# Polochon-street/bliss

Hardware: AMD Instinct MI355X
Metric: songs/sec bl_analyze (3-min 44.1kHz s16) + 10k x 10k distance-matrix sec (higher is better)
Workload: dtype f64; 1 GPU; configs[2] shard: 8192 synthetic 180-s 44.1 kHz s16 stereo songs/GPU resident (260.1 GB), 8192 total; step = analyze + all-gather + row-block distance; songs_per_gpu=8192, parallelism=shard1, fir_mode=2

## Files before the change

### bliss_amd/csrc/bl_env_kernels.hip

```cpp
#include <hip/hip_runtime.h>
#include <atomic>
#include <algorithm>
#include <stdlib.h>

#include "bl_launch.h"
#include "bl_fft_tan.h"
#include "bl_metric.h"
#include "bl_fir.h"
#include "bl_tail.h"

#define EV_CWAVES 7
#define EV_TILE (4 * EV_CWAVES)
#define EV_TROW 258

template <int CTRL> __device__ __forceinline__ double bl_dpp_f64(double v) {
  const unsigned long long b = __double_as_longlong(v);
  const int lo = __builtin_amdgcn_update_dpp(0, (int)(unsigned)(b & 0xFFFFFFFFull), CTRL, 0xF, 0xF, true);
  const int hi = __builtin_amdgcn_update_dpp(0, (int)(unsigned)(b >> 32), CTRL, 0xF, 0xF, true);
  return __longlong_as_double(((unsigned long long)(unsigned)hi << 32) | (unsigned)lo);
}

template <int CTRL> __device__ __forceinline__ double bl_dpp_f64_old(double old, double v) {
  const unsigned long long b = __double_as_longlong(v), o = __double_as_longlong(old);
  const int lo = __builtin_amdgcn_update_dpp((int)(unsigned)(o & 0xFFFFFFFFull), (int)(unsigned)(b & 0xFFFFFFFFull),
// ... 131 lines not shown
        if (ln == 0) flags[8] = st;
        psum = sum;
        if (live && !own) {
          energies[sg.env_off + w] = sum;
          lc[sg.env_off + w] = bl_tail_compress((double)sum, tb.log101);
        }
        stamp(st - 1, 2);
      }
    }
    return;
  }

  auto phase = [&](int k) {
    const int pr = (PRIO >> (4 * k)) & 3;
    if (pr == 0) __builtin_amdgcn_s_setprio(0);
    else if (pr == 1) __builtin_amdgcn_s_setprio(1);
    else if (pr == 2) __builtin_amdgcn_s_setprio(2);
    else __builtin_amdgcn_s_setprio(3);
  };
  double *buf = reinterpret_cast<double *>(smem) + wave * EV3_SLOTS;
  const int mean = st.mean;
  const double rcp = st.rcp, rcp_lo = st.rcp_lo;
  const double kappa = st.kappa;
  auto nrm = [&](int k) -> double { return FIR_MODE == 2 ? (double)k : bl_norm(k, rcp, rcp_lo); };
  const int r0 = run_begin(u0 + wave), r1 = run_begin(u0 + wave + 1);
  constexpr bool EV3_TAN = FIR_MODE != 0;
  double t1[16];
  bl_fft16_fold<double> fold;
  c2d w1r[16];
  if (EV3_TAN) {
    const bl_fft_tan_lane<double> *tl = reinterpret_cast<const bl_fft_tan_lane<double> *>(tb.tan_lane) + l;
    t1[0] = 0.0;
#pragma unroll
    for (int k1 = 1; k1 < 16; ++k1) {
      t1[k1] = tl->t1[k1];
      asm volatile("" : "+v"(t1[k1]));
    }
    fold = tl->fold;
#define EV3_PIN(A, N) _Pragma("unroll") for (int i = 0; i < N; ++i) asm volatile("" : "+v"(A[i]));
    EV3_PIN(fold.rb, 4) EV3_PIN(fold.rc, 4) EV3_PIN(fold.rd, 4) EV3_PIN(fold.fb, 4) EV3_PIN(fold.fc, 2) EV3_PIN(fold.g, 3)
#undef EV3_PIN
  } else {
#pragma unroll
    for (int k1 = 1; k1 < 16; ++k1) {
      w1r[k1] = tw256[k1 * 16 + l];
      asm volatile("" : "+v"(w1r[k1].re), "+v"(w1r[k1].im));
    }
  }
  typedef int ev_v4i __attribute__((ext_vector_type(4)));
  unsigned cp[4][2];
  ev_v4i ini0, ini2, ini4;
  if (FIR_MODE == 2) {
    bl_firi_tap_planes(l, g, cp);
#pragma unroll
    for (int j = 0; j < 4; ++j) asm volatile("" : "+v"(cp[j][0]), "+v"(cp[j][1]));
    int k0, k2, k4;
    bl_firi_const(mean, &k0, &k2, &k4);
    ini0 = ev_v4i{k0, k0, k0, k0};
    ini2 = ev_v4i{k2, k2, k2, k2};
    ini4 = ev_v4i{k4, k4, k4, k4};
  }
  int base5 = (4 * r0) % 5;

  if (r0 < r1) {
    const int s0 = 1024 * r0 + 4 * ln;
    double r[20];
#pragma unroll
    for (int u = 0; u < 5; ++u) {
      const int i0 = s0 - 16 + 4 * u;
      const bool ok = i0 >= 0 && i0 + 4 <= n_used;
      const uint2 v = *reinterpret_cast<const uint2 *>(p + (ok ? i0 : 0));
      const unsigned w[2] = {ok ? v.x : 0u, ok ? v.y : 0u};
#pragma unroll
      for (int k = 0; k < 2; ++k) {
        const int lo = (int)(short)(w[k] & 0xFFFFu), hi = (int)(short)(w[k] >> 16);
        r[4 * u + 2 * k] = ok ? nrm(lo - mean) : 0.0;
        r[4 * u + 2 * k + 1] = ok ? nrm(hi - mean) : 0.0;
      }
    }
    double *dst = buf + base5 * EV3_BLK + EV3_ROW(ln >> 2) + EV3_UNIT(2 * (ln & 3));
#pragma unroll
    for (int i = 0; i < 4; ++i) {
#define XW(m) r[i + 16 - (m)]
      dst[EV3_UNIT(i >> 1) + (i & 1)] = BL_FIR_SEL(FIR_MODE, XW);
#undef XW
    }
  }

  uint4 pre[4];
  short preh;
#if defined(__HIP_DEVICE_COMPILE__) && !defined(__gfx950__)
#error "k_env_windows3: the raw-buffer descriptor and its range check are written for gfx950"
#endif
  const __amdgpu_buffer_rsrc_t prs =
      __builtin_amdgcn_make_buffer_rsrc(const_cast<int16_t *>(p), 0, (int)(2u * (unsigned)n_used), 0x00020000);
  unsigned voff = 2u * (unsigned)(1024 * r0 + 240 + (FIR_MODE == 2 ? 16 * l + 8 * g : 16 * ln));
  unsigned voffh = 2u * (unsigned)(1024 * r0 + 256 * g + l);
  typedef unsigned ev_v4u __attribute__((__vector_size__(16)));
  auto fetch = [&]() {
#pragma unroll
    for (int u = 0; u < 4; ++u) {
      const ev_v4u v = __builtin_amdgcn_raw_buffer_load_b128(prs, (int)(voff + (FIR_MODE == 2 ? 512u : 16u) * u), 0, 0);
      pre[u] = make_uint4(v[0], v[1], v[2], v[3]);
    }
    preh = (short)__builtin_amdgcn_raw_buffer_load_b16(prs, (int)voffh, 0, 0);
    voff += 2048u;
    voffh += 2048u;
  };
  fetch();
  double held[8];
#pragma unroll
  for (int k0 = 0; k0 < 8; ++k0) held[k0] = 0.0;
  auto publish_held_only = [&]() {
    while (__builtin_amdgcn_readfirstlane(flags[8]) < seq - 1) __builtin_amdgcn_s_sleep(1);
    ev_lds_acquire();
    double *tg = terms + (4 * wave + g) * EV_TROW;
#pragma unroll
    for (int k0 = 0; k0 < 8; ++k0)
      if (k0 < 7 || l != 15) tg[256 - l - 16 * k0] = held[k0];
    ev_wave_sync();
  };
  for (int s = 0; s < steps; ++s) {
    ++seq;
    const int rho = r0 + s;
    if (rho >= r1) {
      publish_held_only();
      if (ln == 0) flags[wave] = seq;
      continue;
    }
    stamp(s, 0);
    phase(0);
    double yv[16], yh;
    const int kh = (int)preh - mean;
    if (FIR_MODE == 2) {
      ev_v4i acc[4][5];
#pragma unroll
      for (int t = 0; t < 4; ++t) {
        const unsigned w[4] = {pre[t].x, pre[t].y, pre[t].z, pre[t].w};
        unsigned lp[2], hp[2];
        bl_firi_sample_planes(w, lp, hp);
        const ev_v4i smp = {(int)lp[0], (int)lp[1], (int)hp[0], (int)hp[1]};
        const ev_v4i zero = {0, 0, 0, 0};
#define EV3_W64(A, B) (long)(((unsigned long long)(B) << 32) | (unsigned long long)(A))
#define EV3_TAP2(J) ev_v4i{(int)cp[(J) + 1][0], (int)cp[(J) + 1][1], (int)cp[J][0], (int)cp[J][1]}
        acc[t][0] = __builtin_amdgcn_mfma_i32_16x16x32_i8(EV3_W64(cp[0][0], cp[0][1]), EV3_W64(lp[0], lp[1]), ini0, 0, 0, 0);
        acc[t][1] = __builtin_amdgcn_mfma_i32_16x16x64_i8(EV3_TAP2(0), smp, zero, 0, 0, 0);
        acc[t][2] = __builtin_amdgcn_mfma_i32_16x16x64_i8(EV3_TAP2(1), smp, ini2, 0, 0, 0);
        acc[t][3] = __builtin_amdgcn_mfma_i32_16x16x64_i8(EV3_TAP2(2), smp, zero, 0, 0, 0);
        acc[t][4] = __builtin_amdgcn_mfma_i32_16x16x32_i8(EV3_W64(cp[3][0], cp[3][1]), EV3_W64(hp[0], hp[1]), ini4, 0, 0, 0);
#undef EV3_W64
#undef EV3_TAP2
      }
      fetch();
#pragma unroll
      for (int t = 0; t < 4; ++t)
#pragma unroll
        for (int r = 0; r < 4; ++r)
          yv[4 * t + r] = bl_firi_combine(acc[t][0][r], acc[t][1][r], acc[t][2][r], acc[t][3][r], acc[t][4][r]);
#define KH(m) __builtin_amdgcn_update_dpp(0, kh, 0x110 + (m), 0xF, 0xF, true)
      const double hp_[9] = {(double)kh ,
                             (double)(KH(1) + KH(15)), (double)(KH(2) + KH(14)), (double)(KH(3) + KH(13)),
                             (double)(KH(4) + KH(12)), (double)(KH(5) + KH(11)), (double)(KH(6) + KH(10)),
                             (double)(KH(7) + KH(9)), (double)KH(8)};
#undef KH
#define XP(m) hp_[m]
      yh = BL_FIR_INT_P(XP);
#undef XP
    } else {
      double r[32];
#pragma unroll
      for (int u = 0; u < 4; ++u) {
        const unsigned w[4] = {pre[u].x, pre[u].y, pre[u].z, pre[u].w};
#pragma unroll
        for (int k = 0; k < 4; ++k) {
          const int lo = (int)(short)(w[k] & 0xFFFFu), hi = (int)(short)(w[k] >> 16);
          r[8 * u + 2 * k] = nrm(lo - mean);
          r[8 * u + 2 * k + 1] = nrm(hi - mean);
        }
      }
      const double xh = nrm(kh);
      fetch();
#pragma unroll
      for (int i = 0; i < 16; ++i) {
#define XR(m) r[i + 16 - (m)]
        yv[i] = BL_FIR_SEL(FIR_MODE, XR);
#undef XR
      }
      double hx[17];
      hx[0] = xh;
      hx[1] = bl_dpp_f64<0x111>(xh);  hx[2] = bl_dpp_f64<0x112>(xh);  hx[3] = bl_dpp_f64<0x113>(xh);
      hx[4] = bl_dpp_f64<0x114>(xh);  hx[5] = bl_dpp_f64<0x115>(xh);  hx[6] = bl_dpp_f64<0x116>(xh);
      hx[7] = bl_dpp_f64<0x117>(xh);  hx[8] = bl_dpp_f64<0x118>(xh);  hx[9] = bl_dpp_f64<0x119>(xh);
      hx[10] = bl_dpp_f64<0x11A>(xh); hx[11] = bl_dpp_f64<0x11B>(xh); hx[12] = bl_dpp_f64<0x11C>(xh);
      hx[13] = bl_dpp_f64<0x11D>(xh); hx[14] = bl_dpp_f64<0x11E>(xh); hx[15] = bl_dpp_f64<0x11F>(xh);
      hx[16] = 0.0;
#define XH(m) hx[m]
      yh = BL_FIR_SEL(FIR_MODE, XH);
#undef XH
    }
    const int xa = base5 + g, xb = xa + 1;
    const int pa = xa >= 5 ? xa - 5 : xa, pb = xb >= 5 ? xb - 5 : xb;
    double *blk_a = buf + pa * EV3_BLK, *blk_b = buf + pb * EV3_BLK;
    stamp(s, 1);
    phase(1);
    ev_wave_sync();
    if (FIR_MODE == 2) {
#pragma unroll
      for (int t = 0; t < 4; ++t) {
        const int xt = base5 + t + 1, pt = xt >= 5 ? xt - 5 : xt;
        double *d = buf + pt * EV3_BLK + EV3_ROW(l) + EV3_UNIT(2 * g);
#pragma unroll
        for (int r = 0; r < 4; ++r) d[EV3_UNIT(r >> 1) + (r & 1)] = yv[4 * t + r];
      }
    } else {
#pragma unroll
      for (int i = 0; i < 16; ++i) blk_b[EV3_ROW(l) + EV3_UNIT(i >> 1) + (i & 1)] = yv[i];
    }
    buf[EV3_HEADS + ln] = yh;
    ev_wave_sync();
    double re[16], im[16];
    {
      const int off = EV3_ROW(l >> 3) + EV3_UNIT(l & 7);
      const double *ia = blk_a + off, *ib = blk_b + off;
      const double *i0 = l < 8 ? buf + EV3_HEADS + 16 * g + 2 * l : ia;
      re[0] = i0[0];
      im[0] = i0[1];
#pragma unroll
      for (int m1 = 1; m1 < 8; ++m1) { re[m1] = ia[EV3_ROW(2 * m1)]; im[m1] = ia[EV3_ROW(2 * m1) + 1]; }
#pragma unroll
      for (int m1 = 8; m1 < 16; ++m1) { re[m1] = ib[EV3_ROW(2 * (m1 - 8))]; im[m1] = ib[EV3_ROW(2 * (m1 - 8)) + 1]; }
    }
    ev_wave_sync();
    stamp(s, 2);
    phase(2);
    if (EV3_TAN) {
      bl_fft512_pass1_tan(re, im, t1);
    } else {
      bl_fft16(re, im);
#pragma unroll
      for (int k1 = 1; k1 < 16; ++k1) bl_cmul(re[bl_pos16(k1)], im[bl_pos16(k1)], w1r[k1].re, w1r[k1].im);
    }
    stamp(s, 3);
    phase(3);
    double *xg = blk_a;
    const double2 *xrow = reinterpret_cast<const double2 *>(xg + l * 18);
#pragma unroll
    for (int k1 = 0; k1 < 16; ++k1) xg[k1 * 18 + l] = re[bl_pos16(k1)];
    ev_wave_sync();
#pragma unroll
    for (int q = 0; q < 8; ++q) { const double2 v = xrow[q]; re[2 * q] = v.x; re[2 * q + 1] = v.y; }
    ev_wave_sync();
#pragma unroll
    for (int k1 = 0; k1 < 16; ++k1) xg[k1 * 18 + l] = im[bl_pos16(k1)];
    ev_wave_sync();
#pragma unroll
    for (int q = 0; q < 8; ++q) { const double2 v = xrow[q]; im[2 * q] = v.x; im[2 * q + 1] = v.y; }
    ev_wave_sync();
    stamp(s, 4);
    phase(4);
    double *tg = terms + (4 * wave + g) * EV_TROW;
    stamp(s, 5);
    phase(5);
    while (__builtin_amdgcn_readfirstlane(flags[8]) < seq - 1) {}
    ev_lds_acquire();
    stamp(s, 6);
#pragma unroll
    for (int k0 = 0; k0 < 8; ++k0)
      if (k0 < 7 || l != 15) tg[256 - l - 16 * k0] = held[k0];
    if (EV3_TAN) bl_fft16_folded(re, im, fold);
    else bl_fft16(re, im);
    double mir7 = 0.0;
#pragma unroll
    for (int k0 = 0; k0 < 8; ++k0) {
      const double sr = re[bl_pos16(15 - k0)], si = im[bl_pos16(15 - k0)];
      const double zr = k0 ? re[bl_pos16(16 - k0)] : re[bl_pos16(0)];
      const double zi = k0 ? im[bl_pos16(16 - k0)] : im[bl_pos16(0)];
      const double pr = bl_dpp_f64_old<0x111>(zr, bl_dpp_f64<0x140>(sr));
      const double pi = bl_dpp_f64_old<0x111>(zi, bl_dpp_f64<0x140>(si));
      double own;
      if (FIR_MODE == 2)
        bl_fft512_power1_sq<double>(re[bl_pos16(k0)], im[bl_pos16(k0)], pr, pi, tw512[l + 16 * k0], kappa, own, held[k0]);
      else if (EV3_TAN)
        bl_fft512_power1_tan<double, false>(re[bl_pos16(k0)], im[bl_pos16(k0)], pr, pi, tw512[l + 16 * k0], own, held[k0]);
      else
        bl_fft512_power1<double, false>(re[bl_pos16(k0)], im[bl_pos16(k0)], pr, pi, tw512[l + 16 * k0], own, held[k0]);
      tg[l + 16 * k0] = own;
      if (k0 == 7) mir7 = held[7];
    }
    const double mr = re[bl_pos16(8)], mi = im[bl_pos16(8)];
    const double mid = (FIR_MODE == 2 ? 2.0 * kappa : 4.0) * __builtin_fma(mr, mr, mi * mi);
    if (l == 0) tg[128] = mid;
    if (l == 15) tg[129] = mir7;
    ev_wave_sync();
    if (ln == 0) flags[wave] = seq;
    stamp(s, 7);
    base5 = base5 == 0 ? 4 : base5 - 1;
  }
  ++seq;
  publish_held_only();
  if (ln == 0) flags[wave] = seq;
}

#define BL_TAIL_OMAX 48

__global__ __launch_bounds__(192) void k_env_tail(const bl_dsong *__restrict__ songs,
                                                  const double *__restrict__ lc, int n_songs,
                                                  bl_amd_song_result *res, int what) {
  __shared__ double yblk[2][38 * 64];
  __shared__ double oblk[2][BL_TAIL_OMAX * 64];
  __shared__ int ocnt[2][64];
  __shared__ double rings_ab[29 * 64];
  __shared__ double rings_c[19 * 64];
  __shared__ int flag_mem[4];
  typedef __attribute__((address_space(3))) volatile int lds_vint;
  lds_vint *flags = (lds_vint *)flag_mem;
  __builtin_amdgcn_s_setprio(3);
  const int wave = __builtin_amdgcn_readfirstlane(threadIdx.x >> 6), lane = threadIdx.x & 63;
  const int song = blockIdx.x * 64 + lane;
  const bool valid = song < n_songs;
  bl_dsong sg;
  if (valid) sg = songs[song];
  else { sg.nb_frames = 0; sg.n_windows = 0; sg.env_off = 0; sg.n = 1; sg.duration = 1; }
  const int N = 2 * sg.nb_frames;
  int maxN = N;
#pragma unroll
  for (int off = 32; off > 0; off >>= 1) maxN = max(maxN, __shfl_xor(maxN, off));
  if (threadIdx.x < 4) flags[threadIdx.x] = 0;
  __syncthreads();
  const int n_blocks = (maxN + 37) / 38;

  if (wave == 0) {
    bl_tail_iir a;
    a.init();
    const double *mylc = lc + sg.env_off;
    const int nw = sg.n_windows;
    auto fetch = [&](int kb_, double (&dst)[19]) {
#pragma unroll
      for (int q = 0; q < 19; ++q) dst[q] = mylc[max(min(19 * kb_ + q, nw - 1), 0)];
    };
    auto block = [&](int kb, double (&cur)[19], double (&fut)[19]) {
      if (kb >= n_blocks) return;
      fetch(kb + 2, fut);
      double *yo = yblk[kb & 1] + lane;
      double ye[38];
#pragma unroll
      for (int q = 0; q < 19; ++q) a.pair(19 * kb + q < nw ? cur[q] : 0.0, ye[2 * q], ye[2 * q + 1]);
      while (__builtin_amdgcn_readfirstlane(flags[1]) < kb - 1) __builtin_amdgcn_s_sleep(1);
      ev_lds_acquire();
#pragma unroll
      for (int q = 0; q < 38; ++q) yo[q * 64] = ye[q];
      ev_lds_release();
      bl_wave_sync();
      if (lane == 0) flags[0] = kb + 1;
    };
    double pa[19], pb[19], pc[19];
    fetch(0, pa);
    fetch(1, pb);
    for (int kb = 0; kb < n_blocks; kb += 3) {
      block(kb, pa, pc);
      block(kb + 1, pb, pa);
      block(kb + 2, pc, pb);
    }
    return;
  }

  if (wave == 1) {
    bl_tail_ab t;
    t.init(sg.nb_frames, rings_ab + lane, 64);
    for (int kb = 0; kb < n_blocks; ++kb) {
      while (__builtin_amdgcn_readfirstlane(flags[0]) < kb + 1) __builtin_amdgcn_s_sleep(1);
      while (__builtin_amdgcn_readfirstlane(flags[3]) < kb - 1) __builtin_amdgcn_s_sleep(1);
      ev_lds_acquire();
      const double *yin = yblk[kb & 1] + lane;
      const int j = 38 * kb;
      bl_tail_fifo f;
      f.base = oblk[kb & 1] + lane;
      f.stride = 64;
      f.count = 0;
      if (bl_tail_ab::chunk_ok(j, N)) {
        t.fast_chunk38(yin, 64, f.base, 64);
        f.count = 38;
      } else if (j < N) {
        for (int q = 0; q < 38; ++q) {
          const int jj = j + q;
          if (jj < N) {
            t.step(jj, yin[q * 64], f);
            if (jj == N - 1) t.finish(f);
          }
        }
      }
      ocnt[kb & 1][lane] = f.count;
      ev_lds_release();
      bl_wave_sync();
      if (lane == 0) { flags[1] = kb + 1; flags[2] = kb + 1; }
    }
    if (valid) {
      bl_amd_song_result *r = res + sg.out_idx;
      r->atk_sum = t.atk;
      r->v.attack = bl_tail_attack(t.atk, sg.n);
    }
    return;
  }

  bl_tail_c c;
  c.init(sg.nb_frames, rings_c + lane, 64);
  for (int kb = 0; kb < n_blocks; ++kb) {
    while (__builtin_amdgcn_readfirstlane(flags[2]) < kb + 1) __builtin_amdgcn_s_sleep(1);
    ev_lds_acquire();
    const double *oin = oblk[kb & 1] + lane;
    const int cnt = ocnt[kb & 1][lane];
    if (cnt == 38 && c.chunk_ok()) {
      c.fast_chunk38(oin, 64);
    } else {
      for (int q = 0; q < BL_TAIL_OMAX; ++q)
        if (q < cnt) c.push(oin[q * 64]);
    }
    if (valid && c.taken == N && cnt > 0) c.finish();
    ev_lds_release();
    bl_wave_sync();
    if (lane == 0) flags[3] = kb + 1;
  }
  if (!valid) return;
  bl_amd_song_result *r = res + sg.out_idx;
  r->beat = c.beat();
  r->v.tempo = bl_tail_tempo(c.beat(), sg.duration);
  (void)what;
}


static long long *g_env_probe = nullptr;
#ifdef BL_AMD_MEASURE

static int g_env_variant = -1;
extern "C" __attribute__((visibility("default"))) int bl_amd_measure_env(int variant, void *d_probe) {
  g_env_variant = variant;
  g_env_probe = static_cast<long long *>(d_probe);
  return BL_OK;
}
#endif

static std::atomic<int> g_fir_mode{-1};
int blk_fir_mode() {
  int m = g_fir_mode.load(std::memory_order_relaxed);
  if (m < 0) {
    const char *e = getenv("BL_AMD_FIR_FUSED");
    m = e && *e ? atoi(e) : BL_FIR_FUSED_DEFAULT;
  }
  return m < 0 || m > 2 ? BL_FIR_FUSED_DEFAULT : m;
}
extern "C" int bl_amd_fir_mode(void) { return blk_fir_mode(); }
extern "C" int bl_amd_set_fir_mode(int mode) {
  if (mode < -1 || mode > 2) return BL_UNEXPECTED;
  g_fir_mode.store(mode, std::memory_order_relaxed);
  return BL_OK;
}

#define EV_X_BOTH(T) EV_X(2, T, false) EV_X(2, T, true)
#ifdef BL_AMD_MEASURE
#define EV_INSTANCES EV_X(0, BL_ENV_PRIO, false) EV_X(1, BL_ENV_PRIO, false) EV_X_BOTH(BL_ENV_PRIO) EV_PRIO_TABS(EV_X_BOTH)
#else
#define EV_INSTANCES EV_X(0, BL_ENV_PRIO, false) EV_X(1, BL_ENV_PRIO, false) EV_X(2, BL_ENV_PRIO, false)
#endif

int blk_env_configure_device(void) {
#define EV_X(M, T, P)                                                                                    \
  BL_HIP_CHECK(hipFuncSetAttribute(reinterpret_cast<const void *>(k_env_windows3<M, T, P>),              \
                                   hipFuncAttributeMaxDynamicSharedMemorySize, EV3_LDS_BYTES));
  EV_INSTANCES
#undef EV_X
  return BL_OK;
}

int blk_env_windows(const blk_analyze_args &a, int fir_mode, int first, int count, int maxn) {
  Mark m(a.mark, a.mark_user, PK_ENV, a.stream);
  const int gx2 = grid_x_for(std::max(1, (2 * (maxn / 512)) / (4 * 4 * EV_CWAVES)), count, 2, a.n_cu);
  const dim3 grid(gx2, count), block(64 * (EV_CWAVES + 1));
  int prio = BL_ENV_PRIO;
  bool probe = false;
#ifdef BL_AMD_MEASURE
  if (fir_mode == 2 && g_env_variant >= 0) {
    prio = g_env_variant & 0xFFFFFF;
    probe = (g_env_variant >> 24) != 0;
  }
#endif
#define EV_X(M, T, P)                                                                                    \
  if (fir_mode == (M) && prio == (T) && probe == (P)) {                                                  \
    hipLaunchKernelGGL((k_env_windows3<M, T, P>), grid, block, EV3_LDS_BYTES, a.stream, a.pcm,           \
                       a.songs + first, a.stats + first, a.tb, a.energies, a.lc, g_env_probe);           \
    return BL_OK;                                                                                        \
  }
  EV_INSTANCES
#undef EV_X
  return BL_UNEXPECTED;
}

void blk_env_tail(const blk_analyze_args &a, hipStream_t s, int first, int count) {
  Mark m(a.mark, a.mark_user, PK_TAIL, s);
  hipLaunchKernelGGL(k_env_tail, dim3((count + 63) / 64), dim3(192), 0, s, a.songs + first, a.lc, count,
                     a.results, a.what);
}
```

### bliss_amd/csrc/bl_tail.h

```cpp
#ifndef BL_TAIL_H_
#define BL_TAIL_H_

#if defined(__HIPCC__)
#include <hip/hip_runtime.h>
#define BL_THD __host__ __device__ __forceinline__
#else
#include <math.h>
#define BL_THD inline
#endif

#define BL_BOX 19
#define BL_BOX_HALF 10

#define BL_BUT_B0 1.9510e-05
#define BL_BUT_B1 1.1706e-04
#define BL_BUT_B2 2.9266e-04
#define BL_BUT_B3 3.9021e-04
#define BL_BUT_A0 1.00000
#define BL_BUT_A1 (-4.59007)
#define BL_BUT_A2 8.91034
#define BL_BUT_A3 (-9.34191)
#define BL_BUT_A4 5.56998
#define BL_BUT_A5 (-1.78845)
#define BL_BUT_A6 0.24136

BL_THD double bl_div_const(double x, double c, double rc) {
  const double q0 = x * rc;
  const double r0 = __builtin_fma(-q0, c, x);
  return __builtin_fma(r0, rc, q0);
}
#define BL_DIV19(x) bl_div_const((x), 19.0, 1.0 / 19.0)
#define BL_DIV10(x) bl_div_const((x), 10.0, 1.0 / 10.0)

struct bl_peaks {
  double p1, p2;
  int beat, i;
  BL_THD void init() { p1 = 0; p2 = 0; beat = 0; i = 0; }
  BL_THD void push(double v) {
    if (i >= 2) {
      const float epsilon = 0.000001f;
      double dl = p1 - p2, dr = p1 - v;
      if (dl > epsilon && dr > epsilon) beat++;
    }
    p2 = p1;
    p1 = v;
    ++i;
  }
};

template <bool KEEP_OLD> struct bl_box19 {
  double run;
  int N, t, s19, s10;
  BL_THD void init(int n) { run = 0; N = n; t = 0; s19 = 0; s10 = 0; }

  template <typename SINK>
  BL_THD void push(double v, double old, double *ring, double *olds, int stride, SINK &sink) {
    if (t < BL_BOX) {
      run += v;
    } else {
      run -= ring[s19 * stride];
      run += v;
    }
    ring[s19 * stride] = v;
    if (KEEP_OLD) olds[s10 * stride] = old;
    if (t <= 8) {
      sink.push(BL_DIV19(old));
    } else if (t >= BL_BOX - 1 && t <= N - 2) {
      sink.push(BL_DIV19(run));
    }
    ++t;
    s19 = s19 == BL_BOX - 1 ? 0 : s19 + 1;
    s10 = s10 == 9 ? 0 : s10 + 1;
  }

  template <typename SINK>
  BL_THD void finish(const double *ring, const double *olds, int stride, SINK &sink) {
    double acc = KEEP_OLD ? olds[((N - 10) % 10) * stride] : 0.0;
    for (int k = N - BL_BOX; k < N; ++k) acc += ring[(k % BL_BOX) * stride];
    sink.push(BL_DIV19(acc));
    for (int i = N - 9; i < N; ++i) {
      double old = KEEP_OLD ? olds[(i % 10) * stride] : 0.0;
      sink.push(BL_DIV19(old));
    }
  }
};

struct bl_tail_stage2 {
  bl_box19<false> box;
  bl_peaks peaks;
  double *ring;
  int stride;
  BL_THD void push(double v) { box.push(v, 0.0, ring, (double *)0, stride, peaks); }
};

struct bl_tail {
  double x1, x2, x3, x4, x5, x6;
  double y1, y2, y3, y4, y5, y6;
  double atk;
  bl_box19<true> box1;
  bl_tail_stage2 st2;
  double *ring1, *olds1;
  int stride, N;

  BL_THD void init(int nb_frames, double *scratch, int stride_) {
    x1 = x2 = x3 = x4 = x5 = x6 = 0;
    y1 = y2 = y3 = y4 = y5 = y6 = 0;
    atk = 0;
    N = 2 * nb_frames;
    stride = stride_;
    ring1 = scratch;
    olds1 = scratch + 19 * stride_;
    st2.ring = scratch + 29 * stride_;
    st2.stride = stride_;
    box1.init(N);
    st2.box.init(N);
    st2.peaks.init();
  }

  BL_THD void step(int j, double x) {
    double d = 0;
    d += BL_BUT_B0 * x;
    d += BL_BUT_B1 * x1;
    d += BL_BUT_B2 * x2;
    d += BL_BUT_B3 * x3;
    d += BL_BUT_B2 * x4;
    d += BL_BUT_B1 * x5;
    d += BL_BUT_B0 * x6;
    double c = 0;
    c += BL_BUT_A1 * y1;
    c += BL_BUT_A2 * y2;
    c += BL_BUT_A3 * y3;
    c += BL_BUT_A4 * y4;
    c += BL_BUT_A5 * y5;
    c += BL_BUT_A6 * y6;
    const double y = (d - c) / BL_BUT_A0;
    double dj;
    if (j == 0) dj = y;
    else { dj = y - y1; dj = dj > 0 ? dj : 0; }
    const float lambda = 0.8f;
    const double wa = (1 - lambda) * y + BL_DIV10(lambda * 172 * dj);
    x6 = x5; x5 = x4; x4 = x3; x3 = x2; x2 = x1; x1 = x;
    y6 = y5; y5 = y4; y4 = y3; y3 = y2; y2 = y1; y1 = y;
    double ss = 0;
    if (j <= N - 2) { atk += wa; ss = wa; }
    box1.push(ss, wa, ring1, olds1, stride, st2);
  }

  BL_THD void finish() {
    box1.finish(ring1, olds1, stride, st2);
    st2.box.finish(st2.ring, (const double *)0, stride, st2.peaks);
  }

  BL_THD int beat() const { return st2.peaks.beat; }
};

struct bl_tail_iir {
  double x2, x4, x6;
  double y1, y2, y3, y4, y5, y6;
  BL_THD void init() { x2 = x4 = x6 = 0; y1 = y2 = y3 = y4 = y5 = y6 = 0; }
  BL_THD double feedback(double d) {
    double c = 0;
    c += BL_BUT_A1 * y1;
    c += BL_BUT_A2 * y2;
    c += BL_BUT_A3 * y3;
    c += BL_BUT_A4 * y4;
    c += BL_BUT_A5 * y5;
    c += BL_BUT_A6 * y6;
    const double y = (d - c) / BL_BUT_A0;
    y6 = y5; y5 = y4; y4 = y3; y3 = y2; y2 = y1; y1 = y;
    return y;
  }
  BL_THD void pair(double x, double &y_even, double &y_odd) {
    double d = BL_BUT_B0 * x;
    d += BL_BUT_B2 * x2;
    d += BL_BUT_B2 * x4;
    d += BL_BUT_B0 * x6;
    y_even = feedback(d);
    double e = BL_BUT_B1 * x;
    e += BL_BUT_B3 * x2;
    e += BL_BUT_B1 * x4;
    y_odd = feedback(e);
    x6 = x4; x4 = x2; x2 = x;
  }
};

struct bl_tail_fifo {
  double *base;
  int stride, count;
  BL_THD void push(double v) {
    base[count * stride] = v;
    ++count;
  }
};

struct bl_tail_ab {
  double yp;
  double atk;
  bl_box19<true> box1;
  double *ring1, *olds1;
  int stride, N;

  BL_THD void init(int nb_frames, double *scratch, int stride_) {
    yp = 0;
    atk = 0;
    N = 2 * nb_frames;
    stride = stride_;
    ring1 = scratch;
    olds1 = scratch + 19 * stride_;
    box1.init(N);
  }

  BL_THD static bool steady(int j, int n) { return (j & 1) == 0 && j >= 40 && j + 1 <= n - 12; }
  BL_THD static bool chunk_ok(int j, int n) { return steady(j, n) && steady(j + 36, n); }

  BL_THD double weighted(double y, double dj) {
    const float lambda = 0.8f;
    return (1 - lambda) * y + BL_DIV10(lambda * 172 * dj);
  }

  template <typename SINK> BL_THD void step(int j, double y, SINK &sink) {
    double dj;
    if (j == 0) dj = y;
    else { dj = y - yp; dj = dj > 0 ? dj : 0; }
    const double wa = weighted(y, dj);
    yp = y;
    double ss = 0;
    if (j <= N - 2) { atk += wa; ss = wa; }
    box1.push(ss, wa, ring1, olds1, stride, sink);
  }
  template <typename SINK> BL_THD void finish(SINK &sink) { box1.finish(ring1, olds1, stride, sink); }

  template <int P> BL_THD double stage_a(double y) {
    double dj = y - yp;
    dj = dj > 0 ? dj : 0;
    const double wa = weighted(y, dj);
    yp = y;
    atk += wa;
    return wa;
  }
  template <int P> BL_THD double stage_b(double wa, double (&ra)[BL_BOX]) {
    box1.run -= ra[P];
    box1.run += wa;
    ra[P] = wa;
    return BL_DIV19(box1.run);
  }
  template <int T>
  BL_THD void reg_pipe(const double *yin, int ystride, double *o1out, int ostride, double (&ra)[BL_BOX],
                       double (&wa)[2]) {
    if constexpr (T < 2 * BL_BOX + 1) {
      if constexpr (T >= 1) o1out[(T - 1) * ostride] = stage_b<(T - 1) % BL_BOX>(wa[(T - 1) % 2], ra);
      if constexpr (T < 2 * BL_BOX) wa[T % 2] = stage_a<T % BL_BOX>(yin[T * ystride]);
      reg_pipe<T + 1>(yin, ystride, o1out, ostride, ra, wa);
    }
  }

  BL_THD void fast_chunk38(const double *yin, int ystride, double *o1out, int ostride) {
    double ra[BL_BOX];
    {
      int sa = box1.s19;
#pragma unroll
      for (int k = 0; k < BL_BOX; ++k) {
        ra[k] = ring1[sa * stride];
        sa = sa == BL_BOX - 1 ? 0 : sa + 1;
      }
    }
    double wa[2];
    reg_pipe<0>(yin, ystride, o1out, ostride, ra, wa);
    {
      int sa = box1.s19;
#pragma unroll
      for (int k = 0; k < BL_BOX; ++k) {
        ring1[sa * stride] = ra[k];
        sa = sa == BL_BOX - 1 ? 0 : sa + 1;
      }
    }
    box1.t += 38;
    box1.s10 = (box1.s10 + 8) % 10;
  }
};

struct bl_tail_c {
  bl_box19<false> box;
  bl_peaks peaks;
  double *ring;
  int stride, N, taken;

  BL_THD void init(int nb_frames, double *scratch, int stride_) {
    N = 2 * nb_frames;
    stride = stride_;
    ring = scratch;
    taken = 0;
    box.init(N);
    peaks.init();
  }
  BL_THD void push(double v) {
    box.push(v, 0.0, ring, (double *)0, stride, peaks);
    ++taken;
  }
  BL_THD void finish() { box.finish(ring, (const double *)0, stride, peaks); }
  BL_THD int beat() const { return peaks.beat; }

  BL_THD bool chunk_ok() const { return taken >= BL_BOX && taken + 37 <= N - 2; }

  template <int P> BL_THD void stage_c(double o1, double (&rb)[BL_BOX]) {
    box.run -= rb[P];
    box.run += o1;
    rb[P] = o1;
    const double o2 = BL_DIV19(box.run);
    const float epsilon = 0.000001f;
    const double dl = peaks.p1 - peaks.p2, dr = peaks.p1 - o2;
    peaks.beat += (dl > epsilon && dr > epsilon) ? 1 : 0;
    peaks.p2 = peaks.p1;
    peaks.p1 = o2;
  }
  template <int T> BL_THD void reg_steps(const double *o1in, int istride, double (&rb)[BL_BOX]) {
    if constexpr (T < 2 * BL_BOX) {
      stage_c<T % BL_BOX>(o1in[T * istride], rb);
      reg_steps<T + 1>(o1in, istride, rb);
    }
  }
  BL_THD void fast_chunk38(const double *o1in, int istride) {
    double rb[BL_BOX];
    {
      int sb = box.s19;
#pragma unroll
      for (int k = 0; k < BL_BOX; ++k) {
        rb[k] = ring[sb * stride];
        sb = sb == BL_BOX - 1 ? 0 : sb + 1;
      }
    }
    reg_steps<0>(o1in, istride, rb);
    {
      int sb = box.s19;
#pragma unroll
      for (int k = 0; k < BL_BOX; ++k) {
        ring[sb * stride] = rb[k];
        sb = sb == BL_BOX - 1 ? 0 : sb + 1;
      }
    }
    box.t += 38;
    box.s10 = (box.s10 + 8) % 10;
    peaks.i += 38;
    taken += 38;
  }
};

BL_THD double bl_tail_compress(double f, double log101) {
  const float mu = 100.0f;
  return log(1 + mu * f) / log101;
}

BL_THD float bl_tail_tempo(int beat, unsigned long long duration) {
  return (float)(4 * (float)beat / (float)duration - 30.4);
}
BL_THD float bl_tail_attack(double atk_sum, int n_samples) {
  return (float)(-1.74 * atk_sum * 10000 / n_samples + 58.3);
}

#endif
```

Measured before the change: 26530 songs/s.

## Split envelope tail into five-wave pipeline with shared ring buffers

```diff
diff --git a/bliss_amd/csrc/bl_env_kernels.hip b/bliss_amd/csrc/bl_env_kernels.hip
--- a/bliss_amd/csrc/bl_env_kernels.hip
+++ b/bliss_amd/csrc/bl_env_kernels.hip
@@ -457,18 +457,44 @@
 }
 
 #define BL_TAIL_OMAX 48
-
-__global__ __launch_bounds__(192) void k_env_tail(const bl_dsong *__restrict__ songs,
-                                                  const double *__restrict__ lc, int n_songs,
-                                                  bl_amd_song_result *res, int what) {
-  __shared__ double yblk[2][38 * 64];
-  __shared__ double oblk[2][BL_TAIL_OMAX * 64];
-  __shared__ int ocnt[2][64];
-  __shared__ double rings_ab[29 * 64];
-  __shared__ double rings_c[19 * 64];
-  __shared__ int flag_mem[4];
+enum { TW_FF = 0, TW_FB = 1, TW_A = 2, TW_C = 3, TW_B = 4, TW_WAVES = 5 };
+enum { TF_D = 0, TF_Y, TF_W, TF_O, TF_OC, TF_WORDS = 8 };
+#define BL_TAIL_BUFS 5
+#define TAIL_MARK(S) asm volatile("; tail-budget " S ::: "memory")
+
+struct tail_lds {
+  double sblk[BL_TAIL_BUFS][38 * 64];
+  double oflush[10 * 64];
+  double rings_b[29 * 64];
+  double rings_c[19 * 64];
+  int ocnt[BL_TAIL_BUFS][64];
+  int flags[TF_WORDS];
+};
+static_assert(sizeof(tail_lds) + 2 * (BL_HIST_BINS + 8) * sizeof(float) <= 160 * 1024, "k_env_tail: LDS");
+
+struct tail_o1_sink {
+  double *base, *flush;
+  int count;
+  __device__ __forceinline__ void push(double v) {
+    (count < 38 ? base + count * 64 : flush + (count - 38) * 64)[0] = v;
+    ++count;
+  }
+};
+
+__global__ __launch_bounds__(64 * TW_WAVES) void k_env_tail(const bl_dsong *__restrict__ songs,
+                                                            const double *__restrict__ lc, int n_songs,
+                                                            bl_amd_song_result *res, int what) {
+  __shared__ tail_lds L;
   typedef __attribute__((address_space(3))) volatile int lds_vint;
-  lds_vint *flags = (lds_vint *)flag_mem;
+  lds_vint *flags = (lds_vint *)L.flags;
+  auto wait_for = [&](int word, int seq) {
+    while (__builtin_amdgcn_readfirstlane(flags[word]) < seq) __builtin_amdgcn_s_sleep(1);
+  };
+  auto publish = [&](int lane_, int word, int seq) {
+    ev_lds_release();
+    bl_wave_sync();
+    if (lane_ == 0) flags[word] = seq;
+  };
   __builtin_amdgcn_s_setprio(3);
   const int wave = __builtin_amdgcn_readfirstlane(threadIdx.x >> 6), lane = threadIdx.x & 63;
   const int song = blockIdx.x * 64 + lane;
@@ -480,12 +506,12 @@
   int maxN = N;
 #pragma unroll
   for (int off = 32; off > 0; off >>= 1) maxN = max(maxN, __shfl_xor(maxN, off));
-  if (threadIdx.x < 4) flags[threadIdx.x] = 0;
+  if (threadIdx.x < TF_WORDS) flags[threadIdx.x] = 0;
   __syncthreads();
   const int n_blocks = (maxN + 37) / 38;
 
-  if (wave == 0) {
-    bl_tail_iir a;
+  if (wave == TW_FF) {
+    bl_tail_ff a;
     a.init();
     const double *mylc = lc + sg.env_off;
     const int nw = sg.n_windows;
@@ -493,20 +519,24 @@
 #pragma unroll
       for (int q = 0; q < 19; ++q) dst[q] = mylc[max(min(19 * kb_ + q, nw - 1), 0)];
     };
+    int buf = 0;
     auto block = [&](int kb, double (&cur)[19], double (&fut)[19]) {
       if (kb >= n_blocks) return;
+      TAIL_MARK("FF begin");
       fetch(kb + 2, fut);
-      double *yo = yblk[kb & 1] + lane;
-      double ye[38];
-#pragma unroll
-      for (int q = 0; q < 19; ++q) a.pair(19 * kb + q < nw ? cur[q] : 0.0, ye[2 * q], ye[2 * q + 1]);
-      while (__builtin_amdgcn_readfirstlane(flags[1]) < kb - 1) __builtin_amdgcn_s_sleep(1);
+      double *po = L.sblk[buf] + lane;
+      buf = buf == BL_TAIL_BUFS - 1 ? 0 : buf + 1;
+      wait_for(TF_OC, kb - (BL_TAIL_BUFS - 1));
       ev_lds_acquire();
 #pragma unroll
-      for (int q = 0; q < 38; ++q) yo[q * 64] = ye[q];
-      ev_lds_release();
-      bl_wave_sync();
-      if (lane == 0) flags[0] = kb + 1;
+      for (int q = 0; q < 19; ++q) {
+        double d, e;
+        a.pair(19 * kb + q < nw ? cur[q] : 0.0, d, e);
+        po[2 * q * 64] = d;
+        po[(2 * q + 1) * 64] = e;
+      }
+      publish(lane, TF_D, kb + 1);
+      TAIL_MARK("FF end");
     };
     double pa[19], pb[19], pc[19];
     fetch(0, pa);
@@ -519,35 +549,56 @@
     return;
   }
 
-  if (wave == 1) {
-    bl_tail_ab t;
-    t.init(sg.nb_frames, rings_ab + lane, 64);
-    for (int kb = 0; kb < n_blocks; ++kb) {
-      while (__builtin_amdgcn_readfirstlane(flags[0]) < kb + 1) __builtin_amdgcn_s_sleep(1);
-      while (__builtin_amdgcn_readfirstlane(flags[3]) < kb - 1) __builtin_amdgcn_s_sleep(1);
+  if (wave == TW_FB) {
+    bl_tail_fb r;
+    r.init();
+    for (int kb = 0, buf = 0; kb < n_blocks; ++kb, buf = buf == BL_TAIL_BUFS - 1 ? 0 : buf + 1) {
+      wait_for(TF_D, kb + 1);
       ev_lds_acquire();
-      const double *yin = yblk[kb & 1] + lane;
+      TAIL_MARK("FB begin");
+      double *py = L.sblk[buf] + lane;
+      double ye[38];
+#pragma unroll
+      for (int q = 0; q < 38; ++q) ye[q] = py[q * 64];
+#pragma unroll
+      for (int q = 0; q < 38; ++q) ye[q] = r.step(ye[q]);
+#pragma unroll
+      for (int q = 0; q < 38; ++q) py[q * 64] = ye[q];
+      publish(lane, TF_Y, kb + 1);
+      TAIL_MARK("FB end");
+    }
+    return;
+  }
+
+  if (wave == TW_A) {
+    bl_tail_a t;
+    t.init(sg.nb_frames);
+    for (int kb = 0, buf = 0; kb < n_blocks; ++kb, buf = buf == BL_TAIL_BUFS - 1 ? 0 : buf + 1) {
+      wait_for(TF_Y, kb + 1);
+      ev_lds_acquire();
+      double *pw = L.sblk[buf] + lane;
       const int j = 38 * kb;
-      bl_tail_fifo f;
-      f.base = oblk[kb & 1] + lane;
-      f.stride = 64;
-      f.count = 0;
-      if (bl_tail_ab::chunk_ok(j, N)) {
-        t.fast_chunk38(yin, 64, f.base, 64);
-        f.count = 38;
+      if (bl_tail_a::chunk_ok(j, N)) {
+        TAIL_MARK("A begin");
+        double va[BL_TAIL_G], vb[BL_TAIL_G];
+#pragma unroll
+        for (int q = 0; q < BL_TAIL_G; ++q) va[q] = pw[q * 64];
+#pragma unroll
+        for (int q = 0; q < BL_TAIL_G; ++q) vb[q] = pw[(BL_TAIL_G + q) * 64];
+        t.steady_group(va);
+#pragma unroll
+        for (int q = 0; q < BL_TAIL_G; ++q) pw[q * 64] = va[q];
+        t.steady_group(vb);
+#pragma unroll
+        for (int q = 0; q < BL_TAIL_G; ++q) pw[(BL_TAIL_G + q) * 64] = vb[q];
+        TAIL_MARK("A end");
       } else if (j < N) {
         for (int q = 0; q < 38; ++q) {
           const int jj = j + q;
-          if (jj < N) {
-            t.step(jj, yin[q * 64], f);
-            if (jj == N - 1) t.finish(f);
-          }
+          if (jj < N) pw[q * 64] = t.step(jj, pw[q * 64]);
         }
       }
-      ocnt[kb & 1][lane] = f.count;
-      ev_lds_release();
-      bl_wave_sync();
-      if (lane == 0) { flags[1] = kb + 1; flags[2] = kb + 1; }
+      publish(lane, TF_W, kb + 1);
     }
     if (valid) {
       bl_amd_song_result *r = res + sg.out_idx;
@@ -557,23 +608,71 @@
     return;
   }
 
+  if (wave == TW_B) {
+    bl_tail_b t;
+    t.init(sg.nb_frames, L.rings_b + lane, 64);
+    double ra[BL_BOX] = {};
+    bool in_regs = false;
+    for (int kb = 0, buf = 0; kb < n_blocks; ++kb, buf = buf == BL_TAIL_BUFS - 1 ? 0 : buf + 1) {
+      wait_for(TF_W, kb + 1);
+      ev_lds_acquire();
+      double *win = L.sblk[buf] + lane;
+      const int j = 38 * kb;
+      tail_o1_sink f;
+      f.base = win;
+      f.flush = L.oflush + lane;
+      f.count = 0;
+      const bool steady = bl_tail_b::chunk_ok(j, N);
+      if (steady) {
+        if (!in_regs) t.ring_load(ra);
+        TAIL_MARK("B begin");
+        t.steady38(win, 64, f.base, 64, ra);
+        TAIL_MARK("B end");
+        f.count = 38;
+      } else if (in_regs) {
+        t.ring_store(ra);
+      }
+      in_regs = steady;
+      if (!steady && j < N) {
+        for (int q = 0; q < 38; ++q) {
+          const int jj = j + q;
+          if (jj < N) {
+            t.step(jj, win[q * 64], f);
+            if (jj == N - 1) t.finish(f);
+          }
+        }
+      }
+      L.ocnt[buf][lane] = f.count;
+      publish(lane, TF_O, kb + 1);
+    }
+    return;
+  }
+
   bl_tail_c c;
-  c.init(sg.nb_frames, rings_c + lane, 64);
-  for (int kb = 0; kb < n_blocks; ++kb) {
-    while (__builtin_amdgcn_readfirstlane(flags[2]) < kb + 1) __builtin_amdgcn_s_sleep(1);
+  c.init(sg.nb_frames, L.rings_c + lane, 64);
+  double rb[BL_BOX] = {};
+  bool in_regs = false;
+  for (int kb = 0, buf = 0; kb < n_blocks; ++kb, buf = buf == BL_TAIL_BUFS - 1 ? 0 : buf + 1) {
+    wait_for(TF_O, kb + 1);
     ev_lds_acquire();
-    const double *oin = oblk[kb & 1] + lane;
-    const int cnt = ocnt[kb & 1][lane];
-    if (cnt == 38 && c.chunk_ok()) {
-      c.fast_chunk38(oin, 64);
-    } else {
+    const double *oin = L.sblk[buf] + lane, *ofl = L.oflush + lane;
+    const int cnt = L.ocnt[buf][lane];
+    const bool steady = cnt == 38 && c.chunk_ok();
+    if (steady) {
+      if (!in_regs) c.ring_load(rb);
+      TAIL_MARK("C begin");
+      c.steady38(oin, 64, rb);
+      TAIL_MARK("C end");
+    } else if (in_regs) {
+      c.ring_store(rb);
+    }
+    in_regs = steady;
+    if (!steady) {
       for (int q = 0; q < BL_TAIL_OMAX; ++q)
-        if (q < cnt) c.push(oin[q * 64]);
+        if (q < cnt) c.push(q < 38 ? oin[q * 64] : ofl[(q - 38) * 64]);
     }
     if (valid && c.taken == N && cnt > 0) c.finish();
-    ev_lds_release();
-    bl_wave_sync();
-    if (lane == 0) flags[3] = kb + 1;
+    publish(lane, TF_OC, kb + 1);
   }
   if (!valid) return;
   bl_amd_song_result *r = res + sg.out_idx;
@@ -651,6 +750,6 @@
 
 void blk_env_tail(const blk_analyze_args &a, hipStream_t s, int first, int count) {
   Mark m(a.mark, a.mark_user, PK_TAIL, s);
-  hipLaunchKernelGGL(k_env_tail, dim3((count + 63) / 64), dim3(192), 0, s, a.songs + first, a.lc, count,
+  hipLaunchKernelGGL(k_env_tail, dim3((count + 63) / 64), dim3(64 * TW_WAVES), 0, s, a.songs + first, a.lc, count,
                      a.results, a.what);
 }
diff --git a/bliss_amd/csrc/bl_tail.h b/bliss_amd/csrc/bl_tail.h
--- a/bliss_amd/csrc/bl_tail.h
+++ b/bliss_amd/csrc/bl_tail.h
@@ -31,6 +31,17 @@
 }
 #define BL_DIV19(x) bl_div_const((x), 19.0, 1.0 / 19.0)
 #define BL_DIV10(x) bl_div_const((x), 10.0, 1.0 / 10.0)
+
+#define BL_TAIL_G 19
+BL_THD void bl_div_const_group(double (&x)[BL_TAIL_G], double c, double rc) {
+  double q0[BL_TAIL_G];
+#pragma unroll
+  for (int i = 0; i < BL_TAIL_G; ++i) q0[i] = x[i] * rc;
+#pragma unroll
+  for (int i = 0; i < BL_TAIL_G; ++i) x[i] = __builtin_fma(-q0[i], c, x[i]);
+#pragma unroll
+  for (int i = 0; i < BL_TAIL_G; ++i) x[i] = __builtin_fma(x[i], rc, q0[i]);
+}
 
 struct bl_peaks {
   double p1, p2;
@@ -154,13 +165,28 @@
   BL_THD int beat() const { return st2.peaks.beat; }
 };
 
-struct bl_tail_iir {
+struct bl_tail_ff {
   double x2, x4, x6;
+  BL_THD void init() { x2 = x4 = x6 = 0; }
+  BL_THD void pair(double x, double &d_even, double &d_odd) {
+    double d = BL_BUT_B0 * x;
+    d += BL_BUT_B2 * x2;
+    d += BL_BUT_B2 * x4;
+    d += BL_BUT_B0 * x6;
+    d_even = d;
+    double e = BL_BUT_B1 * x;
+    e += BL_BUT_B3 * x2;
+    e += BL_BUT_B1 * x4;
+    d_odd = e;
+    x6 = x4; x4 = x2; x2 = x;
+  }
+};
+
+struct bl_tail_fb {
   double y1, y2, y3, y4, y5, y6;
-  BL_THD void init() { x2 = x4 = x6 = 0; y1 = y2 = y3 = y4 = y5 = y6 = 0; }
-  BL_THD double feedback(double d) {
-    double c = 0;
-    c += BL_BUT_A1 * y1;
+  BL_THD void init() { y1 = y2 = y3 = y4 = y5 = y6 = 0; }
+  BL_THD double step(double d) {
+    double c = BL_BUT_A1 * y1;
     c += BL_BUT_A2 * y2;
     c += BL_BUT_A3 * y3;
     c += BL_BUT_A4 * y4;
@@ -170,17 +196,17 @@
     y6 = y5; y5 = y4; y4 = y3; y3 = y2; y2 = y1; y1 = y;
     return y;
   }
+};
+
+struct bl_tail_iir {
+  bl_tail_ff ff;
+  bl_tail_fb fb;
+  BL_THD void init() { ff.init(); fb.init(); }
   BL_THD void pair(double x, double &y_even, double &y_odd) {
-    double d = BL_BUT_B0 * x;
-    d += BL_BUT_B2 * x2;
-    d += BL_BUT_B2 * x4;
-    d += BL_BUT_B0 * x6;
-    y_even = feedback(d);
-    double e = BL_BUT_B1 * x;
-    e += BL_BUT_B3 * x2;
-    e += BL_BUT_B1 * x4;
-    y_odd = feedback(e);
-    x6 = x4; x4 = x2; x2 = x;
+    double d, e;
+    ff.pair(x, d, e);
+    y_even = fb.step(d);
+    y_odd = fb.step(e);
   }
 };
 
@@ -193,16 +219,60 @@
   }
 };
 
-struct bl_tail_ab {
+struct bl_tail_a {
   double yp;
   double atk;
+  int N;
+
+  BL_THD void init(int nb_frames) {
+    yp = 0;
+    atk = 0;
+    N = 2 * nb_frames;
+  }
+
+  BL_THD double weighted(double y, double dj) {
+    const float lambda = 0.8f;
+    return (1 - lambda) * y + BL_DIV10(lambda * 172 * dj);
+  }
+
+  BL_THD double step(int j, double y) {
+    double dj;
+    if (j == 0) dj = y;
+    else { dj = y - yp; dj = dj > 0 ? dj : 0; }
+    const double wa = weighted(y, dj);
+    yp = y;
+    if (j <= N - 2) atk += wa;
+    return wa;
+  }
+
+  BL_THD static bool chunk_ok(int j, int n) { return j >= 1 && j + 37 <= n - 2; }
+  BL_THD void steady_group(double (&v)[BL_TAIL_G]) {
+    const float lambda = 0.8f;
+    double t[BL_TAIL_G];
+    t[0] = v[0] - yp;
+#pragma unroll
+    for (int i = 1; i < BL_TAIL_G; ++i) t[i] = v[i] - v[i - 1];
+    yp = v[BL_TAIL_G - 1];
+#pragma unroll
+    for (int i = 0; i < BL_TAIL_G; ++i) t[i] = t[i] > 0 ? t[i] : 0;
+#pragma unroll
+    for (int i = 0; i < BL_TAIL_G; ++i) t[i] = lambda * 172 * t[i];
+    bl_div_const_group(t, 10.0, 1.0 / 10.0);
+#pragma unroll
+    for (int i = 0; i < BL_TAIL_G; ++i) v[i] = (1 - lambda) * v[i];
+#pragma unroll
+    for (int i = 0; i < BL_TAIL_G; ++i) v[i] = v[i] + t[i];
+#pragma unroll
+    for (int i = 0; i < BL_TAIL_G; ++i) atk += v[i];
+  }
+};
+
+struct bl_tail_b {
   bl_box19<true> box1;
   double *ring1, *olds1;
   int stride, N;
 
   BL_THD void init(int nb_frames, double *scratch, int stride_) {
-    yp = 0;
-    atk = 0;
     N = 2 * nb_frames;
     stride = stride_;
     ring1 = scratch;
@@ -213,69 +283,78 @@
   BL_THD static bool steady(int j, int n) { return (j & 1) == 0 && j >= 40 && j + 1 <= n - 12; }
   BL_THD static bool chunk_ok(int j, int n) { return steady(j, n) && steady(j + 36, n); }
 
-  BL_THD double weighted(double y, double dj) {
-    const float lambda = 0.8f;
-    return (1 - lambda) * y + BL_DIV10(lambda * 172 * dj);
-  }
-
-  template <typename SINK> BL_THD void step(int j, double y, SINK &sink) {
-    double dj;
-    if (j == 0) dj = y;
-    else { dj = y - yp; dj = dj > 0 ? dj : 0; }
-    const double wa = weighted(y, dj);
-    yp = y;
-    double ss = 0;
-    if (j <= N - 2) { atk += wa; ss = wa; }
-    box1.push(ss, wa, ring1, olds1, stride, sink);
+  template <typename SINK> BL_THD void step(int j, double wa, SINK &sink) {
+    box1.push(j <= N - 2 ? wa : 0.0, wa, ring1, olds1, stride, sink);
   }
   template <typename SINK> BL_THD void finish(SINK &sink) { box1.finish(ring1, olds1, stride, sink); }
 
-  template <int P> BL_THD double stage_a(double y) {
-    double dj = y - yp;
-    dj = dj > 0 ? dj : 0;
-    const double wa = weighted(y, dj);
-    yp = y;
-    atk += wa;
-    return wa;
-  }
-  template <int P> BL_THD double stage_b(double wa, double (&ra)[BL_BOX]) {
-    box1.run -= ra[P];
-    box1.run += wa;
-    ra[P] = wa;
-    return BL_DIV19(box1.run);
-  }
-  template <int T>
-  BL_THD void reg_pipe(const double *yin, int ystride, double *o1out, int ostride, double (&ra)[BL_BOX],
-                       double (&wa)[2]) {
-    if constexpr (T < 2 * BL_BOX + 1) {
-      if constexpr (T >= 1) o1out[(T - 1) * ostride] = stage_b<(T - 1) % BL_BOX>(wa[(T - 1) % 2], ra);
-      if constexpr (T < 2 * BL_BOX) wa[T % 2] = stage_a<T % BL_BOX>(yin[T * ystride]);
-      reg_pipe<T + 1>(yin, ystride, o1out, ostride, ra, wa);
-    }
-  }
-
-  BL_THD void fast_chunk38(const double *yin, int ystride, double *o1out, int ostride) {
-    double ra[BL_BOX];
-    {
-      int sa = box1.s19;
-#pragma unroll
-      for (int k = 0; k < BL_BOX; ++k) {
-        ra[k] = ring1[sa * stride];
-        sa = sa == BL_BOX - 1 ? 0 : sa + 1;
-      }
-    }
-    double wa[2];
-    reg_pipe<0>(yin, ystride, o1out, ostride, ra, wa);
-    {
-      int sa = box1.s19;
-#pragma unroll
-      for (int k = 0; k < BL_BOX; ++k) {
-        ring1[sa * stride] = ra[k];
-        sa = sa == BL_BOX - 1 ? 0 : sa + 1;
-      }
-    }
+  BL_THD static void ring_turn(double &run, double (&ra)[BL_BOX], double (&v)[BL_BOX]) {
+#pragma unroll
+    for (int i = 0; i < BL_BOX; ++i) {
+      run -= ra[i];
+      run += v[i];
+      ra[i] = v[i];
+      v[i] = run;
+    }
+    bl_div_const_group(v, 19.0, 1.0 / 19.0);
+  }
+
+  BL_THD void ring_load(double (&ra)[BL_BOX]) const {
+    int sa = box1.s19;
+#pragma unroll
+    for (int k = 0; k < BL_BOX; ++k) {
+      ra[k] = ring1[sa * stride];
+      sa = sa == BL_BOX - 1 ? 0 : sa + 1;
+    }
+  }
+  BL_THD void ring_store(const double (&ra)[BL_BOX]) {
+    int sa = box1.s19;
+#pragma unroll
+    for (int k = 0; k < BL_BOX; ++k) {
+      ring1[sa * stride] = ra[k];
+      sa = sa == BL_BOX - 1 ? 0 : sa + 1;
+    }
+  }
+
+  BL_THD void steady38(const double *win, int wstride, double *o1out, int ostride, double (&ra)[BL_BOX]) {
+    double va[BL_BOX], vb[BL_BOX];
+#pragma unroll
+    for (int k = 0; k < BL_BOX; ++k) va[k] = win[k * wstride];
+#pragma unroll
+    for (int k = 0; k < BL_BOX; ++k) vb[k] = win[(BL_BOX + k) * wstride];
+    ring_turn(box1.run, ra, va);
+#pragma unroll
+    for (int k = 0; k < BL_BOX; ++k) o1out[k * ostride] = va[k];
+    ring_turn(box1.run, ra, vb);
+#pragma unroll
+    for (int k = 0; k < BL_BOX; ++k) o1out[(BL_BOX + k) * ostride] = vb[k];
     box1.t += 38;
     box1.s10 = (box1.s10 + 8) % 10;
+  }
+  BL_THD void fast_chunk38(const double *win, int wstride, double *o1out, int ostride) {
+    double ra[BL_BOX];
+    ring_load(ra);
+    steady38(win, wstride, o1out, ostride, ra);
+    ring_store(ra);
+  }
+};
+
+struct bl_tail_ab : bl_tail_a, bl_tail_b {
+  BL_THD void init(int nb_frames, double *scratch, int stride_) {
+    bl_tail_a::init(nb_frames);
+    bl_tail_b::init(nb_frames, scratch, stride_);
+  }
+  BL_THD static bool chunk_ok(int j, int n) { return bl_tail_a::chunk_ok(j, n) && bl_tail_b::chunk_ok(j, n); }
+  template <typename SINK> BL_THD void step(int j, double y, SINK &sink) {
+    bl_tail_b::step(j, bl_tail_a::step(j, y), sink);
+  }
+  BL_THD void fast_chunk38(const double *yin, int ystride, double *o1out, int ostride) {
+    double wa[2][BL_TAIL_G];
+    for (int h = 0; h < 2; ++h) {
+      for (int s = 0; s < BL_TAIL_G; ++s) wa[h][s] = yin[(BL_TAIL_G * h + s) * ystride];
+      steady_group(wa[h]);
+    }
+    bl_tail_b::fast_chunk38(&wa[0][0], 1, o1out, ostride);
   }
 };
 
@@ -302,46 +381,55 @@
 
   BL_THD bool chunk_ok() const { return taken >= BL_BOX && taken + 37 <= N - 2; }
 
-  template <int P> BL_THD void stage_c(double o1, double (&rb)[BL_BOX]) {
-    box.run -= rb[P];
-    box.run += o1;
-    rb[P] = o1;
-    const double o2 = BL_DIV19(box.run);
+  BL_THD void turn_c(double (&rb)[BL_BOX], double (&v)[BL_BOX], double &drp) {
+    bl_tail_b::ring_turn(box.run, rb, v);
     const float epsilon = 0.000001f;
-    const double dl = peaks.p1 - peaks.p2, dr = peaks.p1 - o2;
-    peaks.beat += (dl > epsilon && dr > epsilon) ? 1 : 0;
-    peaks.p2 = peaks.p1;
-    peaks.p1 = o2;
-  }
-  template <int T> BL_THD void reg_steps(const double *o1in, int istride, double (&rb)[BL_BOX]) {
-    if constexpr (T < 2 * BL_BOX) {
-      stage_c<T % BL_BOX>(o1in[T * istride], rb);
-      reg_steps<T + 1>(o1in, istride, rb);
-    }
-  }
-  BL_THD void fast_chunk38(const double *o1in, int istride) {
-    double rb[BL_BOX];
-    {
-      int sb = box.s19;
-#pragma unroll
-      for (int k = 0; k < BL_BOX; ++k) {
-        rb[k] = ring[sb * stride];
-        sb = sb == BL_BOX - 1 ? 0 : sb + 1;
-      }
-    }
-    reg_steps<0>(o1in, istride, rb);
-    {
-      int sb = box.s19;
-#pragma unroll
-      for (int k = 0; k < BL_BOX; ++k) {
-        ring[sb * stride] = rb[k];
-        sb = sb == BL_BOX - 1 ? 0 : sb + 1;
-      }
-    }
+    double dr[BL_BOX];
+    dr[0] = peaks.p1 - v[0];
+#pragma unroll
+    for (int i = 1; i < BL_BOX; ++i) dr[i] = v[i - 1] - v[i];
+    peaks.beat += (drp < -epsilon && dr[0] > epsilon) ? 1 : 0;
+#pragma unroll
+    for (int i = 1; i < BL_BOX; ++i) peaks.beat += (dr[i - 1] < -epsilon && dr[i] > epsilon) ? 1 : 0;
+    drp = dr[BL_BOX - 1];
+    peaks.p2 = v[BL_BOX - 2];
+    peaks.p1 = v[BL_BOX - 1];
+  }
+  BL_THD void ring_load(double (&rb)[BL_BOX]) const {
+    int sb = box.s19;
+#pragma unroll
+    for (int k = 0; k < BL_BOX; ++k) {
+      rb[k] = ring[sb * stride];
+      sb = sb == BL_BOX - 1 ? 0 : sb + 1;
+    }
+  }
+  BL_THD void ring_store(const double (&rb)[BL_BOX]) {
+    int sb = box.s19;
+#pragma unroll
+    for (int k = 0; k < BL_BOX; ++k) {
+      ring[sb * stride] = rb[k];
+      sb = sb == BL_BOX - 1 ? 0 : sb + 1;
+    }
+  }
+  BL_THD void steady38(const double *o1in, int istride, double (&rb)[BL_BOX]) {
+    double va[BL_BOX], vb[BL_BOX];
+#pragma unroll
+    for (int k = 0; k < BL_BOX; ++k) va[k] = o1in[k * istride];
+#pragma unroll
+    for (int k = 0; k < BL_BOX; ++k) vb[k] = o1in[(BL_BOX + k) * istride];
+    double drp = peaks.p2 - peaks.p1;
+    turn_c(rb, va, drp);
+    turn_c(rb, vb, drp);
     box.t += 38;
     box.s10 = (box.s10 + 8) % 10;
     peaks.i += 38;
     taken += 38;
+  }
+  BL_THD void fast_chunk38(const double *o1in, int istride) {
+    double rb[BL_BOX];
+    ring_load(rb);
+    steady38(o1in, istride, rb);
+    ring_store(rb);
   }
 };
 
```

Result: no change. 26610 songs/s (median of 2 runs) (+0.3%).
